# Eric-qi/RDO-PTQ

Measured on AMD Instinct MI355X. Metric: calibration images/sec (Cheng2020 W8A8 task-oriented RDO-PTQ, image-iterations over all units), higher is better.
Workload: dtype f32

## Files before the change

### rdo-ptq_amd/csrc/conv_wgrad.hip

```cpp
#include <utility>

#include "rdo_common.h"

namespace {

typedef float f32x16 __attribute__((ext_vector_type(16)));
typedef float f32x4 __attribute__((ext_vector_type(4)));

constexpr int PK = 32;

struct WgArgs {
    const float* x;
    const float* dy;
    float* slabs;
    int B, H, W, Cin, Ho, Wo, Cout, KH, KW, stride, pad;
    int M, mchunk, nsplit;
    int tiles_co, tiles_ci;
    int square_input;
};

template <int TCO, int TCI, bool VEC>
__global__ __launch_bounds__(256) void conv_wgrad_kernel(WgArgs a) {
    constexpr int WCO = TCO / 2, WCI = TCI / 2;
    constexpr int TM = WCO / 32, TN = WCI / 32;
    constexpr int YQ = TCO / 32, XQ = TCI / 32;
// ... 192 lines not shown
}

int rdo_launch_wgrad_x6(const rdo_conv_desc* d, const float* x, const float* dy, float* slabs, int nsplit, int mchunk, hipStream_t s);
bool rdo_linear_wgrad_h2_ok(const rdo_conv_desc* d, const float* x, const float* dy);
int rdo_launch_linear_wgrad_h2(const rdo_conv_desc* d, const float* x, const float* dy, float* slabs, int nsplit, int mchunk, hipStream_t s);
bool rdo_conv_is_thin(const rdo_conv_desc* d, bool forward);
int rdo_launch_thin_wgrad(const rdo_conv_desc* d, const float* x, const float* dy, float* slabs, int nsplit, hipStream_t s);
bool rdo_conv_is_thincout(const rdo_conv_desc* d, bool forward);
int rdo_thincout_patches(const rdo_conv_desc* d);
int rdo_launch_thincout_wgrad(const rdo_conv_desc* d, const float* x, const float* dy, float* slabs, hipStream_t s);

extern "C" int rdo_conv2d_wgrad_uses_bf16x6(const rdo_conv_desc* d) {
    const bool enabled = rdo::tuning(rdo::T_CONV_X6) != 0;
    if (!d || !enabled || g_force_big == 0) return 0;
    const bool fits = (double)d->B * d->H * d->W * d->Cin * 4.0 < 4.0e9 && (double)d->B * d->Ho * d->Wo * d->Cout * 4.0 < 4.0e9;
    return big_tiles(d) && fits && d->Wo % 4 == 0 && d->Wo >= 16 && d->Cin % 4 == 0 && d->Cout % 4 == 0;
}

extern "C" void rdo_debug_force_wgrad_choice(int big, int nsplit) {
    g_force_big = big;
    g_force_ns = nsplit;
}

extern "C" int rdo_conv2d_wgrad_nsplit(const rdo_conv_desc* d) {
    if (!d) return 1;
    if (g_force_big < 0 && rdo_conv_is_thincout(d, false)) return rdo_thincout_patches(d);
    if (g_force_ns >= 1) return g_force_ns;
    const long M = (long)d->B * d->Ho * d->Wo;
    if (rdo_conv_is_thin(d, false)) {
        const long per = d->KH * d->KW * d->Cin > 4 ? 256 : 512;
        const long cap = d->KH * d->KW * d->Cin > 4 ? 256 : 128;
        const long ns = M / per;
        return (int)(ns < 1 ? 1 : (ns > cap ? cap : ns));
    }
    const long target = big_tiles(d) ? 256 : 1024;
    long ns = target / tiles_total(d);
    const long max_by_m = rdo::ceil_div(M, 128);
    if (ns > max_by_m) ns = max_by_m;
    if (ns < 1) ns = 1;
    const long cap = (g_force_big < 0 && one_tile_many_pixels(d)) ? 256 : ((g_force_big != 0 && rdo_linear_wgrad_h2_ok(d, nullptr, nullptr)) ? 128 : 64);
    if (ns > cap) ns = cap;
    return (int)ns;
}

extern "C" int rdo_conv2d_wgrad(const rdo_conv_desc* d, const float* x, const float* dy, float* slabs, int nsplit,
                                void* stream) {
    RDO_REQUIRE(d && x && dy && slabs, "rdo_conv2d_wgrad: null argument");
    RDO_REQUIRE(nsplit >= 1, "rdo_conv2d_wgrad: nsplit < 1");
    RDO_REQUIRE((long)d->B * d->H * d->W * d->Cin < (1L << 31) && (long)d->B * d->Ho * d->Wo * d->Cout < (1L << 31),
                "rdo_conv2d_wgrad: tensors of 2^31 or more elements are not supported (32-bit staging offsets)");
    WgArgs a;
    a.x = x; a.dy = dy; a.slabs = slabs;
    a.B = d->B; a.H = d->H; a.W = d->W; a.Cin = d->Cin; a.Ho = d->Ho; a.Wo = d->Wo; a.Cout = d->Cout;
    a.KH = d->KH; a.KW = d->KW; a.stride = d->stride; a.pad = d->pad;
    a.M = d->B * d->Ho * d->Wo;
    a.nsplit = nsplit;
    a.mchunk = (int)(rdo::ceil_div(rdo::ceil_div(a.M, nsplit), PK) * PK);
    a.square_input = d->square_input;
    a.tiles_co = a.tiles_ci = 0;
    const bool vec = (d->Cin % 4 == 0) && (d->Cout % 4 == 0) &&
                     ((reinterpret_cast<uintptr_t>(x) | reinterpret_cast<uintptr_t>(dy)) % 16 == 0);
    const bool big = big_tiles(d);
    if (g_force_big < 0 && rdo_conv_is_thincout(d, false) && nsplit == rdo_thincout_patches(d)) {
        const rdo_conv_desc dd = *d;
        return rdo::dispatch([=](hipStream_t s) { return rdo_launch_thincout_wgrad(&dd, x, dy, slabs, s); }, stream, "conv_thincout_wgrad",
// ... 32 lines not shown
```

### rdo-ptq_amd/csrc/conv_wgrad_h2.hip

```cpp
#include <utility>

#include "rdo_common.h"

namespace {

typedef float f32x4acc __attribute__((ext_vector_type(4)));
typedef _Float16 f16x8 __attribute__((ext_vector_type(8)));
typedef short s16x8 __attribute__((ext_vector_type(8)));
typedef short s16x4 __attribute__((ext_vector_type(4)));
constexpr int NP = 2;
typedef unsigned short u16;

__device__ __attribute__((aligned(64))) unsigned g_zero_page_w[16];

constexpr int PK = 32;
constexpr int SUBB = 32 * 128;
constexpr int PLANEB = 3 * SUBB;
constexpr int OPB = NP * PLANEB;
constexpr int STAGEB = 2 * OPB;

struct WgPArgs {
    const u16* xp;
    const u16* yp;
    long xplane, yplane;
    float* slabs;
// ... 409 lines not shown
        Ey = Ex = 0;
    }

    const float fy = lw_pow2(-Ey), fx = lw_pow2(-Ex);
    float* slab = a.slabs + (long)chunk * a.Cout * a.Cin;
#pragma unroll
    for (int j = 0; j < TN; ++j) {
        const int ci = ci0 + wci0 + j * 16 + l16;
        if (ci >= a.Cin) continue;
#pragma unroll
        for (int i = 0; i < TM; ++i)
#pragma unroll
            for (int r = 0; r < 4; ++r) {
                const int co = co0 + wco0 + i * 16 + 4 * lc + r;
                if (co < a.Cout) slab[(long)co * a.Cin + ci] = (acc[i][j][r] * fy) * fx;
            }
    }
}

constexpr int XROWS = 40;
constexpr int XPLANEB = XROWS * 128;
constexpr int STAGE3B = OPB + NP * XPLANEB;

template <int SUB, int RING3, int LSLOT, int PF = 0>
__global__ __launch_bounds__(512, 2) void conv_wgrad_h2r_kernel(WgPArgs a) {
    constexpr int T = 192;
    constexpr int TM = 3, TN = 6;
    constexpr int SLOTB = SUB * STAGE3B;

    extern __shared__ __attribute__((aligned(16))) char smem[];

    const int tid = threadIdx.x, lane = tid & 63, wave = __builtin_amdgcn_readfirstlane(tid >> 6);
    const int l16 = lane & 15, lc = lane >> 4;
    const int wco0 = (wave >> 1) * 48;

    const int nwg = gridDim.x * gridDim.y;
    const int lin = blockIdx.x + gridDim.x * blockIdx.y;
    const int xq = nwg >> 3, xr = nwg & 7, xcd = lin & 7;
    const int lid = (xcd < xr ? xcd * (xq + 1) : xr * (xq + 1) + (xcd - xr) * xq) + (lin >> 3);
    const int chunk = lid / gridDim.y;
    int t = lid - chunk * gridDim.y;
    const int cib = t % a.tiles_ci; t /= a.tiles_ci;
    const int tco = t % a.tiles_co; t /= a.tiles_co;
    const int kh = __builtin_amdgcn_readfirstlane(t);
    const int co0 = tco * T, ci0 = cib * 64;

    const int segs_row = a.Wo / PK;
    const int segs_total = a.B * a.Ho * segs_row;
    const int spc = (segs_total + a.nsplit - 1) / a.nsplit;
    const int sbeg = chunk * spc;
    const int send = min(segs_total, sbeg + spc);
    const int nsegs = send > sbeg ? send - sbeg : 0;
    const int nsteps = (nsegs + SUB - 1) / SUB;

    const int prow8 = (lane >> 1) & 7, dsl = lane >> 4, dhalf = lane & 1;
    constexpr int XP = NP * 5;
    constexpr unsigned OOB = 0xFFFFFFFFu;
    constexpr int RSRC3 = 0x00020000;
    typedef __attribute__((address_space(3))) void lds_void;
    const unsigned ybytes = (unsigned)(a.yplane * 2), xbytes = (unsigned)(a.xplane * 2);
    __amdgpu_buffer_rsrc_t ry[3], rx[2];
    unsigned yvoff[3], xvoff[2];
    int ydst[3], xdst[2];
#pragma unroll
    for (int j = 0; j < 3; ++j) {
        const int k = wave + 8 * j;
        const int plane = k / 12, sub = (k % 12) >> 2, rg = k & 3;
        const int row = 8 * rg + prow8;
        const int ch = co0 + 64 * sub + 16 * dsl + 8 * dhalf;
        ry[j] = __builtin_amdgcn_make_buffer_rsrc((void*)(a.yp + plane * a.yplane), 0, ybytes, RSRC3);
        yvoff[j] = ch < a.Cout ? (unsigned)(((ch >> 4) * a.M + row) * 16 + (ch & 15)) * 2u : OOB;
        ydst[j] = plane * PLANEB + sub * SUBB + rg * 1024;
    }
    int xedge[2];
#pragma unroll
    for (int j = 0; j < 2; ++j) {
        const int k = wave + 8 * j < XP ? wave + 8 * j : wave;
        const int plane = k / 5, rg = k - plane * 5;
        const int row = 8 * rg + prow8;
        const int ch = ci0 + 16 * dsl + 8 * dhalf;
        rx[j] = __builtin_amdgcn_make_buffer_rsrc((void*)(a.xp + plane * a.xplane - 16), 0, xbytes + 32u, RSRC3);
        xvoff[j] = row < PK + 2 ? (unsigned)(((ch >> 4) * a.Min + row) * 16 + (ch & 15)) * 2u : OOB;
        xedge[j] = (row == 0 ? 1 : 0) | (row == PK + 1 ? 2 : 0) | 4;
        xdst[j] = OPB + plane * XPLANEB + rg * 1024;
    }
    int seg = sbeg;
    int cho = (sbeg / segs_row) % a.Ho;
    int cws = sbeg % segs_row;
    unsigned ysoff = (unsigned)sbeg * (PK * 32u);
    unsigned xsoff = (unsigned)(sbeg * PK + (kh - 1) * a.W) * 32u;
    const int row_bad = kh == 0 ? 0 : kh == 2 ? a.Ho - 1 : -1;
    auto dma_seg = [&](char* const dst) {
        const bool live = seg < send;
        const int emask = (cws == 0 ? 1 : 0) | (cws == segs_row - 1 ? 2 : 0) | ((!live || cho == row_bad) ? 4 : 0);
        const unsigned ys = ysoff, xs = xsoff;
        ++seg; ysoff += PK * 32u; xsoff += PK * 32u;
        if (++cws == segs_row) { cws = 0; if (++cho == a.Ho) cho = 0; }
        if (WG_ABL(1)) return;
#pragma unroll
        for (int j = 0; j < 3; ++j)
            __builtin_amdgcn_raw_ptr_buffer_load_lds(ry[j], (lds_void*)(dst + ydst[j]), 16, live ? yvoff[j] : OOB, ys, 0, 0);
#pragma unroll
        for (int j = 0; j < 2; ++j) {
            if (RING3 == 2 && wave + 8 * j >= XP) break;
            __builtin_amdgcn_raw_ptr_buffer_load_lds(rx[j], (lds_void*)(dst + xdst[j]), 16, (xedge[j] & emask) ? OOB : xvoff[j], xs, 0, 0);
        }
    };
    auto dma_stage = [&](int buf) {
#pragma unroll
        for (int u = 0; u < SUB; ++u) dma_seg(smem + buf * SLOTB + u * STAGE3B);
    };

    f32x4acc acc[TM][TN];
#pragma unroll
    for (int i = 0; i < TM; ++i)
#pragma unroll
        for (int j = 0; j < TN; ++j) acc[i][j] = f32x4acc{0.f, 0.f, 0.f, 0.f};

    const int fr = 4 * lc + ((lane >> 2) & 3);
    const int p4 = lane & 3;
    int fa_off[TM], fb_off[TN];
#pragma unroll
    for (int i = 0; i < TM; ++i) {
        const int c = wco0 + 16 * i;
        fa_off[i] = (c >> 6) * SUBB + (fr >> 3) * 1024 + ((c & 63) >> 4) * 256 + (fr & 7) * 32 + p4 * 8;
    }
#pragma unroll
    for (int j = 0; j < TN; ++j) {
        const int jt = 6 * (wave & 1) + j;
        const int row = fr + (jt >> 2);
        fb_off[j] = OPB + (row >> 3) * 1024 + (jt & 3) * 256 + (row & 7) * 32 + p4 * 8;
    }

    constexpr int PA[3] = {1, 0, 0};
    constexpr int PB[3] = {0, 1, 0};

    const bool late = wave >= 4;
    if (nsteps > 0) {
#pragma unroll
        for (int r = 0; r < RING3 - 1; ++r) dma_stage(r);
    }
    if constexpr (PF != 0) {
        static_assert(SUB == 1 && RING3 == 3, "look-ahead variant: one segment per stage, ring of three");
        f16x8 fa[2][NP][TM], fb[2][NP][2];
        auto rd_a = [&](auto pc, const char* st) {
            constexpr int P = decltype(pc)::value;
#pragma unroll
            for (int p = 0; p < NP; ++p)
#pragma unroll
                for (int i = 0; i < TM; ++i) fa[P][p][i] = tr_pair(st + p * PLANEB + fa_off[i]);
        };
        auto rd_b = [&](auto setc, const char* st, int third) {
            constexpr int S = decltype(setc)::value;
#pragma unroll
            for (int p = 0; p < NP; ++p)
#pragma unroll
                for (int j = 0; j < 2; ++j) fb[S][p][j] = tr_pair(st + p * XPLANEB + fb_off[2 * third + j]);
        };
#ifdef RDO_DIAG
        const unsigned long long st_c0 = clock64(), st_r0 = wall_clock64();
#endif
        if (nsteps > 0) {
            asm volatile("s_waitcnt vmcnt(5)" ::: "memory");
            __builtin_amdgcn_s_barrier();
            rd_a(std::integral_constant<int, 0>{}, smem);
            rd_b(std::integral_constant<int, 0>{}, smem, 0);
        }
        auto stage = [&](auto pc, const int s, const int buf) {
            constexpr int P = decltype(pc)::value;
            asm volatile("s_waitcnt vmcnt(0)" ::: "memory");
            __builtin_amdgcn_s_barrier();
            const int nb = buf >= 1 ? buf - 1 : 2;
            const int nx = buf == 2 ? 0 : buf + 1;
            const bool more = s + 2 < nsteps, ahead = s + 1 < nsteps;
            if (more && !late) dma_stage(nb);
            const char* st = smem + buf * SLOTB;
            const char* sn = smem + nx * SLOTB;
            [&]<int... SL>(std::integer_sequence<int, SL...>) {
                (([&] {
                     constexpr int T3 = SL / 3, Q = SL % 3, SET = (T3 + P) & 1;
                     using NS = std::integral_constant<int, SET ^ 1>;
                     if constexpr (Q == 0) {
                         tr_wait();
                         if constexpr (PF == 1) {
                             if constexpr (T3 < 2) rd_b(NS{}, st, T3 + 1);
                             else if (ahead) { rd_a(std::integral_constant<int, P ^ 1>{}, sn); rd_b(NS{}, sn, 0); }
                         }
                     }
                     if constexpr (PF == 1) {
#pragma unroll
                         for (int i = 0; i < TM; ++i)
#pragma unroll
                             for (int j = 0; j < 2; ++j)
                                 acc[i][2 * T3 + j] =
                                     __builtin_amdgcn_mfma_f32_16x16x32_f16(fa[P][PA[Q]][i], fb[SET][PB[Q]][j], acc[i][2 * T3 + j], 0, 0, 0);
                     } else {
                         [&]<int... U>(std::integer_sequence<int, U...>) {
                             (([&] {
                                  constexpr int i = U / 2, j = U % 2, K = Q * 6 + U;
                                  acc[i][2 * T3 + j] =
                                      __builtin_amdgcn_mfma_f32_16x16x32_f16(fa[P][PA[Q]][i], fb[SET][PB[Q]][j], acc[i][2 * T3 + j], 0, 0, 0);
                                  if constexpr (T3 < 2) {
                                      if constexpr (K < 4) fb[SET ^ 1][K / 2][K % 2] = tr_pair(st + (K / 2) * XPLANEB + fb_off[2 * (T3 + 1) + K % 2]);
                                  } else {
                                      if constexpr (K < 6) fa[P ^ 1][K / 3][K % 3] = tr_pair(sn + (K / 3) * PLANEB + fa_off[K % 3]);
                                      else if constexpr (K < 10) fb[SET ^ 1][(K - 6) / 2][(K - 6) % 2] = tr_pair(sn + ((K - 6) / 2) * XPLANEB + fb_off[(K - 6) % 2]);
                                  }
                                  __builtin_amdgcn_sched_barrier(0);
                              }()),
                              ...);
                         }
                         (std::make_integer_sequence<int, 6>{});
                     }
                     __builtin_amdgcn_sched_barrier(0);
                     if constexpr (SL == LSLOT) {
                         if (more && late) dma_stage(nb);
                     }
                     __builtin_amdgcn_sched_barrier(0);
                 }()),
                 ...);
            }
            (std::make_integer_sequence<int, 9>{});
        };
        int buf = 0;
        for (int s = 0; s < nsteps; s += 2) {
            stage(std::integral_constant<int, 0>{}, s, buf);
            buf = buf == 2 ? 0 : buf + 1;
            if (s + 1 < nsteps) {
                stage(std::integral_constant<int, 1>{}, s + 1, buf);
                buf = buf == 2 ? 0 : buf + 1;
            }
        }
        tr_wait();
#ifdef RDO_DIAG
        if (tid == 0 && lin < 256) {
// ... 93 lines not shown
            }
            (std::make_integer_sequence<int, 9>{});
#ifdef RDO_DIAG
            if (phase_on) ph[4] += clock64() - tb;
#endif
        }
        buf = buf + 1 == RING3 ? 0 : buf + 1;
    }
#ifdef RDO_DIAG
    if (tid == 0 && lin < 256) {
        g_wg_stamps[lin * 4 + 0] = clock64() - st_c0; g_wg_stamps[lin * 4 + 1] = wall_clock64() - st_r0;
        g_wg_stamps[lin * 4 + 2] = (unsigned long long)(nsteps * SUB); g_wg_stamps[lin * 4 + 3] = 0;
    }
    if (phase_on && lane == 0 && lin < 256)
        for (int k = 0; k < 6; ++k) g_wg_phase[(lin * 8 + wave) * 8 + k] = ph[k];
#endif
    }
    asm volatile("s_waitcnt vmcnt(0)" ::: "memory");

    const long wsize = (long)a.Cout * 9 * a.Cin;
    float* slab = a.slabs + (long)chunk * wsize;
#pragma unroll
    for (int j = 0; j < TN; ++j) {
        const int jt = 6 * (wave & 1) + j;
        const int tap = kh * 3 + (jt >> 2);
        const int ci = ci0 + (jt & 3) * 16 + l16;
#pragma unroll
        for (int i = 0; i < TM; ++i)
#pragma unroll
            for (int r = 0; r < 4; ++r) {
                const int co = co0 + wco0 + i * 16 + 4 * lc + r;
                if (co < a.Cout) slab[((long)co * 9 + tap) * a.Cin + ci] = acc[i][j][r] * a.inv_scale;
            }
    }
}

}

extern "C" int rdo_conv2d_wgrad_uses_bf16x6(const rdo_conv_desc* d);
extern "C" int rdo_conv2d_wgrad_nsplit(const rdo_conv_desc* d);

extern "C" int rdo_conv2d_wgrad_h2_supported(const rdo_conv_desc* d) {
    if (!d || d->square_input || d->Cin % 16 != 0 || d->Cout % 16 != 0) return 0;
    if ((double)d->B * d->H * d->W * d->Cin >= 2147483648.0 - 64.0 || (double)d->B * d->Ho * d->Wo * d->Cout >= 2147483648.0 - 64.0) return 0;
    return rdo_conv2d_wgrad_uses_bf16x6(d);
}

// ... 16 lines not shown
    a.B = d->B; a.H = d->H; a.W = d->W; a.Cin = d->Cin; a.Ho = d->Ho; a.Wo = d->Wo; a.Cout = d->Cout;
    a.KH = d->KH; a.KW = d->KW; a.stride = d->stride; a.pad = d->pad;
    a.M = d->B * d->Ho * d->Wo;
    a.Min = d->B * d->H * d->W;
    a.xplane = (long)a.Min * a.Cin;
    a.yplane = (long)a.M * a.Cout;
    a.nsplit = nsplit;
    RDO_REQUIRE(x_scale > 0.f && dy_scale > 0.f, "rdo_conv2d_wgrad_h2: scales must be positive powers of two");
    a.inv_scale = 1.f / (x_scale * dy_scale);
#ifdef RDO_DIAG
    a.ablate = rdo::tuning(rdo::T_X6P_ABLATE);
#endif
    long mchunk = rdo::ceil_div(rdo::ceil_div((long)a.M, nsplit), 32) * 32;
    a.mchunk = (int)mchunk;
    RDO_REQUIRE((long)nsplit * mchunk >= a.M, "rdo_conv2d_wgrad_h2: nsplit too small");
    a.tiles_co = (int)rdo::ceil_div(a.Cout, T);
    a.tiles_ci = (int)rdo::ceil_div(a.Cin, T);
    const double flops = 2.0 * a.M * (double)a.Cout * a.Cin * a.KH * a.KW;
    const double bytes = 4.0 * (a.xplane + a.yplane) + 4.0 * nsplit * (double)a.Cout * a.KH * a.KW * a.Cin;
    if (rdo_conv2d_wgrad_h2_supported(d) && rdo::tuning(rdo::T_WGRAD_P3_ROW) && a.KH == 3 && a.KW == 3 && a.stride == 1 && a.pad == 1 && a.Wo % 32 == 0 && a.Cin % 64 == 0 &&
        a.Wo == a.W && a.Ho == a.H && (long)(a.M / 32) >= nsplit) {
        WgPArgs b = a;
        b.tiles_ci = a.Cin / 64;
        const int variant = rdo::tuning(rdo::T_WGRAD_SUB);
        return rdo::dispatch(
            [b, variant](hipStream_t s) {
                auto go = [&](auto subc, auto ringc, auto slotc, auto pfc) -> int {
                    constexpr int SUB = decltype(subc)::value, RING = decltype(ringc)::value, LS = decltype(slotc)::value, PF = decltype(pfc)::value;
                    constexpr size_t lds = (size_t)RING * SUB * STAGE3B;
                    static_assert(lds <= 160 * 1024, "row weight-gradient LDS");
                    static rdo::PerDevice attr;
                    if (!attr.done()) {
                        if (hipFuncSetAttribute(reinterpret_cast<const void*>(conv_wgrad_h2r_kernel<SUB, RING, LS, PF>),
                                                hipFuncAttributeMaxDynamicSharedMemorySize, (int)lds) != hipSuccess)
                            return rdo::set_error(RDO_EHIP, "hipFuncSetAttribute(conv_wgrad_h2r) failed");
                        attr.mark();
                    }
                    dim3 grid((unsigned)b.nsplit, (unsigned)(3 * b.tiles_co * b.tiles_ci));
                    hipLaunchKernelGGL((conv_wgrad_h2r_kernel<SUB, RING, LS, PF>), grid, dim3(512), lds, s, b);
                    return rdo::check_launch("conv_wgrad_h2r");
                };
                using rdo_i1 = std::integral_constant<int, 1>; using rdo_i2 = std::integral_constant<int, 2>; using rdo_i3 = std::integral_constant<int, 3>;
                using rdo_i5 [[maybe_unused]] = std::integral_constant<int, 5>; using rdo_i8 = std::integral_constant<int, 8>;
                using rdo_i0 = std::integral_constant<int, 0>;
                switch (variant) {
                    case 2: return go(rdo_i2{}, rdo_i2{}, rdo_i2{}, rdo_i0{});
                    case 3: return go(rdo_i1{}, rdo_i3{}, rdo_i8{}, rdo_i0{});
                    case 9: return go(rdo_i1{}, rdo_i3{}, rdo_i2{}, rdo_i1{});
                    case 13: return go(rdo_i1{}, rdo_i3{}, rdo_i2{}, rdo_i2{});
#ifdef RDO_DIAG
                    case 4: return go(rdo_i1{}, rdo_i3{}, rdo_i5{}, rdo_i0{});
                    case 5: return go(rdo_i1{}, rdo_i2{}, rdo_i5{}, rdo_i0{});
                    case 6: return go(rdo_i1{}, rdo_i2{}, rdo_i8{}, rdo_i0{});
                    case 7: return go(rdo_i1{}, rdo_i2{}, rdo_i0{}, rdo_i0{});
                    case 8: return go(rdo_i1{}, rdo_i3{}, rdo_i5{}, rdo_i1{});
                    case 10: return go(rdo_i1{}, rdo_i3{}, rdo_i8{}, rdo_i1{});
                    case 11: return go(rdo_i1{}, rdo_i3{}, rdo_i0{}, rdo_i1{});
                    case 12: return go(rdo_i1{}, rdo_i3{}, rdo_i3{}, rdo_i1{});
                    case 14: return go(rdo_i1{}, rdo_i3{}, rdo_i5{}, rdo_i2{});
                    case 15: return go(rdo_i1{}, rdo_i3{}, rdo_i0{}, rdo_i2{});
#endif
                    default: return go(rdo_i1{}, rdo_i2{}, rdo_i2{}, rdo_i0{});
                }
            },
            stream, "conv_wgrad_h2_rows", flops, bytes);
    }
    return rdo::dispatch(
        [a](hipStream_t s) {
            constexpr size_t lds = (size_t)2 * STAGEB;
            static rdo::PerDevice attr;
            if (!attr.done()) {
                if (hipFuncSetAttribute(reinterpret_cast<const void*>(conv_wgrad_h2_kernel), hipFuncAttributeMaxDynamicSharedMemorySize,
                                        (int)lds) != hipSuccess)
                    return rdo::set_error(RDO_EHIP, "hipFuncSetAttribute(conv_wgrad_h2) failed");
                attr.mark();
            }
            dim3 grid((unsigned)a.nsplit, (unsigned)(a.KH * a.KW * a.tiles_co * a.tiles_ci));
            hipLaunchKernelGGL(conv_wgrad_h2_kernel, grid, dim3(512), lds, s, a);
            return rdo::check_launch("conv_wgrad_h2");
        },
        stream, "conv_wgrad_h2_192x192", flops, bytes);
}

static long lw_min_tokens() {
    static const long v = [] { const char* e = getenv("RDO_LIN_WGRAD_H2_MIN"); return e ? atol(e) : 4096L; }();
// ... 43 lines not shown
```

### rdo-ptq_amd/csrc/rdo_common.h

```cpp
#pragma once
#include <hip/hip_runtime.h>

#include <atomic>
#include <cstdarg>
#include <cstdint>
#include <cstdio>
#include <functional>
#include <string>
#include <vector>

#include "../../include/rdo_ptq_hip.h"

namespace rdo {

struct Op {
    std::function<int(hipStream_t)> fn;
    const char* tag;
    double flops;
    double bytes;
};

struct Recorder {
    bool active = false;
    std::vector<Op>* sink = nullptr;
// ... 15 lines not shown
    hipError_t e = hipGetLastError();
    if (e != hipSuccess) return set_error(RDO_EHIP, "%s: %s", what, hipGetErrorString(e));
    return RDO_OK;
}

#define RDO_REQUIRE(cond, ...)                                  \
    do {                                                        \
        if (!(cond)) return rdo::set_error(RDO_EINVAL, __VA_ARGS__); \
    } while (0)

constexpr int kWave = 64;

struct PerDevice {
    std::atomic<uint64_t> bits{0};
    static uint64_t bit() {
        int d = 0;
        (void)hipGetDevice(&d);
        return 1ull << (d & 63);
    }
    bool done() const { return (bits.load(std::memory_order_acquire) & bit()) != 0; }
    void mark() { bits.fetch_or(bit(), std::memory_order_release); }
};

enum Tune { T_WGRAD_X6_W8 = 0, T_CONV_X6, T_FWD_X6_VER, T_XCD, T_X6P_ABLATE, T_GRAPH_UNROLL, T_TAIL_GRID, T_X6P_HALO, T_WGRAD_P3_ROW, T_THIN_MFMA, T_H2_STAGGER, T_ADA_W1_MIN, T_H2_K32, T_WGRAD_SUB, T_H2_N48, T_COUNT };
int tuning(Tune t);

__host__ __device__ inline long frag_index(long e, int Cout, int KH, int KW, int Cin) {
    if (Cin % 16 != 0) return e;
    long t = e / Cin;
    const int ci = (int)(e - t * Cin);
    const int kw = (int)(t % KW);
    t /= KW;
    const int kh = (int)(t % KH);
    const long co = t / KH;
    return (((((long)(ci >> 4) * KH + kh) * KW + kw) * Cout + co) << 4) + (ci & 15);
}
__host__ __device__ inline int group_row(int r, int rows) { return (r & 3) * (rows >> 2) + (r >> 2); }
__host__ __device__ inline long group_row_elem(long e, int rows, long inner) {
    const long r = e / inner;
    return (long)group_row((int)r, rows) * inner + (e - r * inner);
}
inline int64_t ceil_div(int64_t a, int64_t b) { return (a + b - 1) / b; }

constexpr int kGridCap = 2048;
inline unsigned grid_for(long n, int per_thread = 1) {
    const long g = ceil_div(n, 256L * per_thread);
    return (unsigned)(g < 1 ? 1 : (g > kGridCap ? kGridCap : g));
// ... 69 lines not shown
```

### rdo-ptq_amd/csrc/runtime.hip

```cpp
#include "rdo_common.h"

#include <atomic>
#include <cstdlib>
#include <cstring>
#include <mutex>

namespace rdo {

static thread_local std::string g_err;
static thread_local Recorder g_rec;

Recorder& recorder() { return g_rec; }

int set_error(int code, const char* fmt, ...) {
    char buf[512];
    va_list ap;
    va_start(ap, fmt);
    vsnprintf(buf, sizeof buf, fmt, ap);
    va_end(ap);
    g_err = buf;
    return code;
}

namespace {
struct TuneDef { const char* key; const char* env; int dflt; };
constexpr TuneDef kTune[T_COUNT] = {{"wgrad_x6_w8", "RDO_WGX6_W8", 1}, {"conv_x6", "RDO_CONV_X6", 1},
                                    {"fwd_x6_ver", "RDO_X6_VER", 6}, {"xcd", "RDO_XCD", 1},
                                    {"x6p_ablate", "RDO_X6P_ABLATE", 0}, {"graph_unroll", "RDO_GRAPH_UNROLL", 8},
                                    {"tail_grid", "RDO_TAIL_GRID", 1024}, {"x6p_halo", "RDO_X6P_HALO", 1},
                                    {"wgrad_p3_row", "RDO_WGRAD_P3_ROW", 1}, {"thin_mfma", "RDO_THIN_MFMA", 1},
                                    {"h2_stagger", "RDO_H2_STAGGER", 1}, {"ada_w1_min", "RDO_ADA_W1_MIN", 128},
                                    {"h2_k32", "RDO_H2_K32", 3}, {"wgrad_sub", "RDO_WGRAD_SUB", 13}, {"h2_n48", "RDO_H2_N48", 1}};
std::atomic<int> g_tune[T_COUNT];
std::once_flag g_tune_once;
void tune_init() {
    std::call_once(g_tune_once, [] {
        for (int i = 0; i < T_COUNT; ++i) {
            const char* e = getenv(kTune[i].env);
            int v = e ? atoi(e) : kTune[i].dflt;
#ifndef RDO_DIAG
            if (i == T_X6P_ABLATE || (i == T_FWD_X6_VER && v < 5) || (i == T_WGRAD_X6_W8 && v == 0)) v = kTune[i].dflt;
#endif
            g_tune[i].store(v);
        }
    });
}
int tune_index(const char* key) {
    if (!key) return -1;
    for (int i = 0; i < T_COUNT; ++i)
        if (!strcmp(key, kTune[i].key)) return i;
    return -1;
}
}

int tuning(Tune t) {
// ... 291 lines not shown
```

### rdo-ptq_amd/hipops/_lib.py

```python
import ctypes as C
import os

_HERE = os.path.dirname(os.path.abspath(__file__))
LIB_PATH = os.path.join(os.path.dirname(_HERE), "lib", "librdoptq_hip.so")

EPI_NONE, EPI_LRELU, EPI_LRELU_BWD, EPI_GDN, EPI_IGDN, EPI_RELU, EPI_RELU_BWD, EPI_GELU, EPI_GELU_BWD = range(9)
LOG_SLOTS = 32


class ConvDesc(C.Structure):
    _fields_ = [(n, C.c_int32) for n in ("B", "H", "W", "Cin", "Ho", "Wo", "Cout", "KH", "KW", "stride", "pad", "epilogue",
                                         "square_input", "add_residual")]


class AdaDesc(C.Structure):
    _fields_ = [("numel", C.c_int64), ("rows", C.c_int32), ("n_levels", C.c_int32), ("reparam", C.c_int32),
                ("reparam_bound", C.c_float), ("reparam_pedestal", C.c_float), ("KH", C.c_int32), ("KW", C.c_int32),
                ("Cin", C.c_int32)]


class AdaStepItem(C.Structure):
    _fields_ = [("d", AdaDesc), ("w", C.c_void_p), ("delta", C.c_void_p), ("zp", C.c_void_p), ("slabs", C.c_void_p),
                ("nsplit", C.c_int32), ("alpha", C.c_void_p), ("adam_m", C.c_void_p), ("adam_v", C.c_void_p), ("wq", C.c_void_p),
                ("wd", C.c_void_p), ("wq_planes", C.c_void_p), ("wd_planes", C.c_void_p), ("dalpha", C.c_void_p),
# ... 173 lines not shown
    "rdo_uaq_width_scan": (C.c_int, [P, C.c_int32, C.c_int64, C.POINTER(C.c_int32), C.c_int32, P, P, P, P, P, P, P, P]),
    "rdo_uaq_width_scan_workspace": (C.c_int64, [C.c_int32, C.c_int64, C.c_int32]),
}
EXPORTS_BITS = tuple(_SIGS_BITS)
WIDTH_SCAN_MAX_K = 8
WIDTH_SCAN_MIN_BITS, WIDTH_SCAN_MAX_BITS = 2, 16
WIDTH_SCAN_LDS_ROW, WIDTH_SCAN_CHUNK = 8192, 4096
_SIGS_PACK = {
    "rdo_weight_pack": (C.c_int, [P, P, P, P, C.c_int32, C.c_int64, C.c_int32, P, P]),
    "rdo_weight_unpack": (C.c_int, [P, P, P, C.c_int32, C.c_int64, C.c_int32, P, P, P]),
    "rdo_pack_row_words": (C.c_int64, [C.c_int64, C.c_int32]),
}
EXPORTS_PACK = tuple(_SIGS_PACK)
PACK_MIN_BITS, PACK_MAX_BITS = 2, 16

_SIGS_ACTBITS = {
    "rdo_actquant_width_scan": (C.c_int, [P, C.c_int64, C.c_int32, P, C.POINTER(C.c_int32), C.c_int32, P, P, P, P]),
    "rdo_actquant_width_scan_workspace": (C.c_int64, [C.c_int32, C.c_int32]),
}
EXPORTS_ACTBITS = tuple(_SIGS_ACTBITS)
ACT_WIDTH_SCAN_MAX_K = 8
ACT_WIDTH_SCAN_MIN_BITS, ACT_WIDTH_SCAN_MAX_BITS = 2, 16

_lib = None


def lib():
    global _lib
    if _lib is None:
        if not os.path.exists(LIB_PATH):
            raise RuntimeError(f"{LIB_PATH} not found: build it with `python __graft_entry__.py` or "
                               f"`make -C rdo-ptq_amd/csrc` (no CPU fallback exists)")
        import torch
        h = C.CDLL(LIB_PATH)
        for name, (res, args) in (list(_SIGS.items()) + list(_SIGS_GDN.items()) + list(_SIGS_BIAS.items()) + list(_SIGS_BITS.items())
                                  + list(_SIGS_PACK.items()) + list(_SIGS_SUBPEL.items()) + list(_SIGS_ACTBITS.items())):
            fn = getattr(h, name)
            fn.restype, fn.argtypes = res, args
        _lib = h
    return _lib


def check(rc, what=""):
    if rc != 0:
        raise RuntimeError(f"librdoptq_hip {what} failed ({rc}): {lib().rdo_last_error().decode()}")
```

### rdo-ptq_amd/hipops/ops.py

```python
import ctypes as C
import math
import threading

import torch

from . import _args as A
from . import _lib as L


class H2:
    __slots__ = ("t", "scale", "flag")

    def __init__(self, t, scale, flag=None):
        self.t, self.scale = t, float(scale)
        self.flag = flag
        m, e = math.frexp(self.scale)
        if not (self.scale > 0 and m == 0.5):
            raise ValueError(f"H2 scale must be a positive power of two, got {scale}")

    @property
    def device(self):
        return self.t.device


# ... 1517 lines not shown
            "rdo_pixel_shuffle_h2")


def pixel_unshuffle2(x, out=None, out_planes=None):
    B, Hr, Wr, Cc = x.shape
    if out is None and out_planes is None:
        out = torch.empty((B, Hr // 2, Wr // 2, 4 * Cc), device=x.device, dtype=torch.float32)
    _bind_out(out_planes)
    L.check(L.lib().rdo_pixel_unshuffle2(_ptr(x), B, Hr // 2, Wr // 2, Cc, _ptr(out), _ptr(out_planes), _oscale(out_planes), _stream()),
            "rdo_pixel_unshuffle2")
    return out


def wgrad_h2_supported(x_shape, w_shape, stride, pad):
    d = conv_desc(x_shape, w_shape, stride, pad)
    return bool(L.lib().rdo_conv2d_wgrad_h2_supported(C.byref(d)))


def wgrad_h2_layer_supported(x_shape, w_shape, stride, pad):
    d = conv_desc(x_shape, w_shape, stride, pad)
    return bool(L.lib().rdo_conv2d_wgrad_h2_layer_supported(C.byref(d)))


def conv2d_wgrad_h2(xp, x_shape, dyp, w_shape, stride=1, pad=0, slabs=None):
    d = conv_desc(x_shape, w_shape, stride, pad)
    ns = int(L.lib().rdo_conv2d_wgrad_nsplit(C.byref(d))) if slabs is None else slabs.shape[0]
    if slabs is None:
        slabs = torch.empty((ns,) + tuple(w_shape), device=xp.device, dtype=torch.float32)
    L.check(L.lib().rdo_conv2d_wgrad_h2(C.byref(d), _ptr(xp), xp.scale, _ptr(dyp), dyp.scale, _ptr(slabs), ns, _stream()), "rdo_conv2d_wgrad_h2")
    return slabs
```

Before: 21860.

## Add narrow 96-channel output tile variant for row weight-gradient kernel

Adds a TCO=96 template variant of the fp16 row-based 3x3 weight-gradient kernel, where four waves share a 48-column output strip instead of two. A heuristic picks the narrow tile when the 192-wide tiling leaves too few workgroups or too little work per split. The split count is recomputed from the narrower tile count so the grid grows. The aim is better CU occupancy on small or low-Cout layers, at the cost of more x-operand re-loading per output channel and more partial slabs to reduce.

```diff
diff --git a/include/rdo_ptq_wgrad.h b/include/rdo_ptq_wgrad.h
--- /dev/null
+++ b/include/rdo_ptq_wgrad.h
@@ -0,0 +1,15 @@
+#ifndef RDO_PTQ_WGRAD_H
+#define RDO_PTQ_WGRAD_H
+
+#include "rdo_ptq_hip.h"
+
+#ifdef __cplusplus
+extern "C" {
+#endif
+
+int rdo_conv2d_wgrad_h2_tco(const rdo_conv_desc* d);
+
+#ifdef __cplusplus
+}
+#endif
+#endif
diff --git a/rdo-ptq_amd/csrc/conv_wgrad.hip b/rdo-ptq_amd/csrc/conv_wgrad.hip
--- a/rdo-ptq_amd/csrc/conv_wgrad.hip
+++ b/rdo-ptq_amd/csrc/conv_wgrad.hip
@@ -1,6 +1,7 @@
 #include <utility>
 
 #include "rdo_common.h"
+#include "../../include/rdo_ptq_wgrad.h"
 
 namespace {
 
@@ -239,6 +240,34 @@
     g_force_ns = nsplit;
 }
 
+
+static long splits_for_tiles(const rdo_conv_desc* d, long tiles) {
+    const long M = (long)d->B * d->Ho * d->Wo;
+    const long target = big_tiles(d) ? 256 : 1024;
+    long ns = target / tiles;
+    const long max_by_m = rdo::ceil_div(M, 128);
+    if (ns > max_by_m) ns = max_by_m;
+    if (ns < 1) ns = 1;
+    const long cap = (g_force_big < 0 && one_tile_many_pixels(d)) ? 256 : ((g_force_big != 0 && rdo_linear_wgrad_h2_ok(d, nullptr, nullptr)) ? 128 : 64);
+    return ns > cap ? cap : ns;
+}
+
+extern "C" int rdo_conv2d_wgrad_h2_tco(const rdo_conv_desc* d) {
+    const int mode = rdo::tuning(rdo::T_WGRAD_NARROW);
+    if (!d || mode == 0 || g_force_ns >= 1) return 192;
+    const bool rows = d->KH == 3 && d->KW == 3 && d->stride == 1 && d->pad == 1 && d->Wo % 32 == 0 && d->Cin % 64 == 0 && d->Wo == d->W &&
+                      d->Ho == d->H && rdo_conv2d_wgrad_h2_supported(d);
+    if (!rows) return 192;
+    if (mode == 96) return 96;
+    const long segs = (long)d->B * d->Ho * d->Wo / 32;
+    const long ns192 = splits_for_tiles(d, tiles_total(d));
+    if (rdo::ceil_div(segs, ns192) >= 64) return 192;
+    const long tiles96 = 3 * rdo::ceil_div(d->Cout, 96) * (d->Cin / 64);
+    const long ns96 = splits_for_tiles(d, tiles96);
+    if (rdo::ceil_div(segs, ns96) >= 8 && tiles96 * ns96 >= 224) return 96;
+    return 192;
+}
+
 extern "C" int rdo_conv2d_wgrad_nsplit(const rdo_conv_desc* d) {
     if (!d) return 1;
     if (g_force_big < 0 && rdo_conv_is_thincout(d, false)) return rdo_thincout_patches(d);
@@ -250,14 +279,9 @@
         const long ns = M / per;
         return (int)(ns < 1 ? 1 : (ns > cap ? cap : ns));
     }
-    const long target = big_tiles(d) ? 256 : 1024;
-    long ns = target / tiles_total(d);
-    const long max_by_m = rdo::ceil_div(M, 128);
-    if (ns > max_by_m) ns = max_by_m;
-    if (ns < 1) ns = 1;
-    const long cap = (g_force_big < 0 && one_tile_many_pixels(d)) ? 256 : ((g_force_big != 0 && rdo_linear_wgrad_h2_ok(d, nullptr, nullptr)) ? 128 : 64);
-    if (ns > cap) ns = cap;
-    return (int)ns;
+    const int tco = rdo_conv2d_wgrad_h2_tco(d);
+    const long tiles = tco != 192 ? 3 * rdo::ceil_div(d->Cout, tco) * (d->Cin / 64) : (long)tiles_total(d);
+    return (int)splits_for_tiles(d, tiles);
 }
 
 extern "C" int rdo_conv2d_wgrad(const rdo_conv_desc* d, const float* x, const float* dy, float* slabs, int nsplit,
diff --git a/rdo-ptq_amd/csrc/conv_wgrad_h2.hip b/rdo-ptq_amd/csrc/conv_wgrad_h2.hip
--- a/rdo-ptq_amd/csrc/conv_wgrad_h2.hip
+++ b/rdo-ptq_amd/csrc/conv_wgrad_h2.hip
@@ -1,6 +1,7 @@
 #include <utility>
 
 #include "rdo_common.h"
+#include "../../include/rdo_ptq_wgrad.h"
 
 namespace {
 
@@ -456,17 +457,24 @@
 constexpr int XPLANEB = XROWS * 128;
 constexpr int STAGE3B = OPB + NP * XPLANEB;
 
-template <int SUB, int RING3, int LSLOT, int PF = 0>
+template <int SUB, int RING3, int LSLOT, int PF = 0, int TCO = 192>
 __global__ __launch_bounds__(512, 2) void conv_wgrad_h2r_kernel(WgPArgs a) {
-    constexpr int T = 192;
-    constexpr int TM = 3, TN = 6;
-    constexpr int SLOTB = SUB * STAGE3B;
+    static_assert(TCO == 192 || (TCO == 96 && PF == 2), "narrow tiles: the shipped look-ahead stage shape only");
+    constexpr int T = TCO;
+    constexpr int CLOG = TCO == 192 ? 1 : 2;
+    constexpr int TM = 3, TN = 12 >> CLOG;
+    constexpr int CPT = TN / 3;
+    constexpr int YSUBS = (TCO + 63) / 64;
+    constexpr int YPLANEB = YSUBS * SUBB, YOPB = NP * YPLANEB;
+    constexpr int STG = YOPB + NP * XPLANEB;
+    constexpr int YPW = NP * YSUBS * 4 / 8;
+    constexpr int SLOTB = SUB * STG;
 
     extern __shared__ __attribute__((aligned(16))) char smem[];
 
     const int tid = threadIdx.x, lane = tid & 63, wave = __builtin_amdgcn_readfirstlane(tid >> 6);
     const int l16 = lane & 15, lc = lane >> 4;
-    const int wco0 = (wave >> 1) * 48;
+    const int wco0 = (wave >> CLOG) * 48, colg = wave & ((1 << CLOG) - 1);
 
     const int nwg = gridDim.x * gridDim.y;
     const int lin = blockIdx.x + gridDim.x * blockIdx.y;
@@ -497,14 +505,16 @@
     unsigned yvoff[3], xvoff[2];
     int ydst[3], xdst[2];
 #pragma unroll
-    for (int j = 0; j < 3; ++j) {
+    for (int j = 0; j < YPW; ++j) {
         const int k = wave + 8 * j;
-        const int plane = k / 12, sub = (k % 12) >> 2, rg = k & 3;
+        const int plane = k / (4 * YSUBS), sub = (k % (4 * YSUBS)) >> 2, rg = k & 3;
         const int row = 8 * rg + prow8;
         const int ch = co0 + 64 * sub + 16 * dsl + 8 * dhalf;
+        bool chok = ch < a.Cout;
+        if constexpr (TCO % 64 != 0) chok = chok && 64 * sub + 16 * dsl < TCO;
         ry[j] = __builtin_amdgcn_make_buffer_rsrc((void*)(a.yp + plane * a.yplane), 0, ybytes, RSRC3);
-        yvoff[j] = ch < a.Cout ? (unsigned)(((ch >> 4) * a.M + row) * 16 + (ch & 15)) * 2u : OOB;
-        ydst[j] = plane * PLANEB + sub * SUBB + rg * 1024;
+        yvoff[j] = chok ? (unsigned)(((ch >> 4) * a.M + row) * 16 + (ch & 15)) * 2u : OOB;
+        ydst[j] = plane * YPLANEB + sub * SUBB + rg * 1024;
     }
     int xedge[2];
 #pragma unroll
@@ -516,7 +526,7 @@
         rx[j] = __builtin_amdgcn_make_buffer_rsrc((void*)(a.xp + plane * a.xplane - 16), 0, xbytes + 32u, RSRC3);
         xvoff[j] = row < PK + 2 ? (unsigned)(((ch >> 4) * a.Min + row) * 16 + (ch & 15)) * 2u : OOB;
         xedge[j] = (row == 0 ? 1 : 0) | (row == PK + 1 ? 2 : 0) | 4;
-        xdst[j] = OPB + plane * XPLANEB + rg * 1024;
+        xdst[j] = YOPB + plane * XPLANEB + rg * 1024;
     }
     int seg = sbeg;
     int cho = (sbeg / segs_row) % a.Ho;
@@ -532,7 +542,7 @@
         if (++cws == segs_row) { cws = 0; if (++cho == a.Ho) cho = 0; }
         if (WG_ABL(1)) return;
 #pragma unroll
-        for (int j = 0; j < 3; ++j)
+        for (int j = 0; j < YPW; ++j)
             __builtin_amdgcn_raw_ptr_buffer_load_lds(ry[j], (lds_void*)(dst + ydst[j]), 16, live ? yvoff[j] : OOB, ys, 0, 0);
 #pragma unroll
         for (int j = 0; j < 2; ++j) {
@@ -542,7 +552,7 @@
     };
     auto dma_stage = [&](int buf) {
 #pragma unroll
-        for (int u = 0; u < SUB; ++u) dma_seg(smem + buf * SLOTB + u * STAGE3B);
+        for (int u = 0; u < SUB; ++u) dma_seg(smem + buf * SLOTB + u * STG);
     };
 
     f32x4acc acc[TM][TN];
@@ -561,9 +571,9 @@
     }
 #pragma unroll
     for (int j = 0; j < TN; ++j) {
-        const int jt = 6 * (wave & 1) + j;
+        const int jt = TN * colg + j;
         const int row = fr + (jt >> 2);
-        fb_off[j] = OPB + (row >> 3) * 1024 + (jt & 3) * 256 + (row & 7) * 32 + p4 * 8;
+        fb_off[j] = YOPB + (row >> 3) * 1024 + (jt & 3) * 256 + (row & 7) * 32 + p4 * 8;
     }
 
     constexpr int PA[3] = {1, 0, 0};
@@ -576,26 +586,26 @@
     }
     if constexpr (PF != 0) {
         static_assert(SUB == 1 && RING3 == 3, "look-ahead variant: one segment per stage, ring of three");
-        f16x8 fa[2][NP][TM], fb[2][NP][2];
+        f16x8 fa[2][NP][TM], fb[2][NP][CPT];
         auto rd_a = [&](auto pc, const char* st) {
             constexpr int P = decltype(pc)::value;
 #pragma unroll
             for (int p = 0; p < NP; ++p)
 #pragma unroll
-                for (int i = 0; i < TM; ++i) fa[P][p][i] = tr_pair(st + p * PLANEB + fa_off[i]);
+                for (int i = 0; i < TM; ++i) fa[P][p][i] = tr_pair(st + p * YPLANEB + fa_off[i]);
         };
         auto rd_b = [&](auto setc, const char* st, int third) {
             constexpr int S = decltype(setc)::value;
 #pragma unroll
             for (int p = 0; p < NP; ++p)
 #pragma unroll
-                for (int j = 0; j < 2; ++j) fb[S][p][j] = tr_pair(st + p * XPLANEB + fb_off[2 * third + j]);
+                for (int j = 0; j < CPT; ++j) fb[S][p][j] = tr_pair(st + p * XPLANEB + fb_off[CPT * third + j]);
         };
 #ifdef RDO_DIAG
         const unsigned long long st_c0 = clock64(), st_r0 = wall_clock64();
 #endif
         if (nsteps > 0) {
-            asm volatile("s_waitcnt vmcnt(5)" ::: "memory");
+            asm volatile("s_waitcnt vmcnt(%0)" ::"n"(YPW + 2) : "memory");
             __builtin_amdgcn_s_barrier();
             rd_a(std::integral_constant<int, 0>{}, smem);
             rd_b(std::integral_constant<int, 0>{}, smem, 0);
@@ -625,26 +635,27 @@
 #pragma unroll
                          for (int i = 0; i < TM; ++i)
 #pragma unroll
-                             for (int j = 0; j < 2; ++j)
-                                 acc[i][2 * T3 + j] =
-                                     __builtin_amdgcn_mfma_f32_16x16x32_f16(fa[P][PA[Q]][i], fb[SET][PB[Q]][j], acc[i][2 * T3 + j], 0, 0, 0);
+                             for (int j = 0; j < CPT; ++j)
+                                 acc[i][CPT * T3 + j] =
+                                     __builtin_amdgcn_mfma_f32_16x16x32_f16(fa[P][PA[Q]][i], fb[SET][PB[Q]][j], acc[i][CPT * T3 + j], 0, 0, 0);
                      } else {
+                         constexpr int MPS = TM * CPT, NB = NP * CPT;
                          [&]<int... U>(std::integer_sequence<int, U...>) {
                              (([&] {
-                                  constexpr int i = U / 2, j = U % 2, K = Q * 6 + U;
-                                  acc[i][2 * T3 + j] =
-                                      __builtin_amdgcn_mfma_f32_16x16x32_f16(fa[P][PA[Q]][i], fb[SET][PB[Q]][j], acc[i][2 * T3 + j], 0, 0, 0);
+                                  constexpr int i = U / CPT, j = U % CPT, K = Q * MPS + U;
+                                  acc[i][CPT * T3 + j] =
+                                      __builtin_amdgcn_mfma_f32_16x16x32_f16(fa[P][PA[Q]][i], fb[SET][PB[Q]][j], acc[i][CPT * T3 + j], 0, 0, 0);
                                   if constexpr (T3 < 2) {
-                                      if constexpr (K < 4) fb[SET ^ 1][K / 2][K % 2] = tr_pair(st + (K / 2) * XPLANEB + fb_off[2 * (T3 + 1) + K % 2]);
+                                      if constexpr (K < NB) fb[SET ^ 1][K / CPT][K % CPT] = tr_pair(st + (K / CPT) * XPLANEB + fb_off[CPT * (T3 + 1) + K % CPT]);
                                   } else {
-                                      if constexpr (K < 6) fa[P ^ 1][K / 3][K % 3] = tr_pair(sn + (K / 3) * PLANEB + fa_off[K % 3]);
-                                      else if constexpr (K < 10) fb[SET ^ 1][(K - 6) / 2][(K - 6) % 2] = tr_pair(sn + ((K - 6) / 2) * XPLANEB + fb_off[(K - 6) % 2]);
+                                      if constexpr (K < 6) fa[P ^ 1][K / 3][K % 3] = tr_pair(sn + (K / 3) * YPLANEB + fa_off[K % 3]);
+                                      else if constexpr (K < 6 + NB) fb[SET ^ 1][(K - 6) / CPT][(K - 6) % CPT] = tr_pair(sn + ((K - 6) / CPT) * XPLANEB + fb_off[(K - 6) % CPT]);
                                   }
                                   __builtin_amdgcn_sched_barrier(0);
                               }()),
                               ...);
                          }
-                         (std::make_integer_sequence<int, 6>{});
+                         (std::make_integer_sequence<int, MPS>{});
                      }
                      __builtin_amdgcn_sched_barrier(0);
                      if constexpr (SL == LSLOT) {
@@ -784,7 +795,7 @@
     float* slab = a.slabs + (long)chunk * wsize;
 #pragma unroll
     for (int j = 0; j < TN; ++j) {
-        const int jt = 6 * (wave & 1) + j;
+        const int jt = TN * colg + j;
         const int tap = kh * 3 + (jt >> 2);
         const int ci = ci0 + (jt & 3) * 16 + l16;
 #pragma unroll
@@ -847,45 +858,50 @@
         a.Wo == a.W && a.Ho == a.H && (long)(a.M / 32) >= nsplit) {
         WgPArgs b = a;
         b.tiles_ci = a.Cin / 64;
-        const int variant = rdo::tuning(rdo::T_WGRAD_SUB);
+        const int tco = rdo_conv2d_wgrad_h2_tco(d);
+        b.tiles_co = (int)rdo::ceil_div(a.Cout, tco);
+        const int variant = tco == 192 ? rdo::tuning(rdo::T_WGRAD_SUB) : -96;
         return rdo::dispatch(
             [b, variant](hipStream_t s) {
-                auto go = [&](auto subc, auto ringc, auto slotc, auto pfc) -> int {
+                auto go = [&](auto subc, auto ringc, auto slotc, auto pfc, auto tcoc) -> int {
                     constexpr int SUB = decltype(subc)::value, RING = decltype(ringc)::value, LS = decltype(slotc)::value, PF = decltype(pfc)::value;
-                    constexpr size_t lds = (size_t)RING * SUB * STAGE3B;
-                    static_assert(lds <= 160 * 1024, "row weight-gradient LDS");
+                    constexpr int TCO = decltype(tcoc)::value;
+                    constexpr size_t lds = (size_t)RING * SUB * (NP * ((TCO + 63) / 64) * SUBB + NP * XPLANEB);
+                    static_assert(lds <= 160 * 1024 && (TCO != 192 || lds == (size_t)RING * SUB * STAGE3B), "row weight-gradient LDS");
                     static rdo::PerDevice attr;
                     if (!attr.done()) {
-                        if (hipFuncSetAttribute(reinterpret_cast<const void*>(conv_wgrad_h2r_kernel<SUB, RING, LS, PF>),
+                        if (hipFuncSetAttribute(reinterpret_cast<const void*>(conv_wgrad_h2r_kernel<SUB, RING, LS, PF, TCO>),
                                                 hipFuncAttributeMaxDynamicSharedMemorySize, (int)lds) != hipSuccess)
                             return rdo::set_error(RDO_EHIP, "hipFuncSetAttribute(conv_wgrad_h2r) failed");
                         attr.mark();
                     }
                     dim3 grid((unsigned)b.nsplit, (unsigned)(3 * b.tiles_co * b.tiles_ci));
-                    hipLaunchKernelGGL((conv_wgrad_h2r_kernel<SUB, RING, LS, PF>), grid, dim3(512), lds, s, b);
+                    hipLaunchKernelGGL((conv_wgrad_h2r_kernel<SUB, RING, LS, PF, TCO>), grid, dim3(512), lds, s, b);
                     return rdo::check_launch("conv_wgrad_h2r");
                 };
                 using rdo_i1 = std::integral_constant<int, 1>; using rdo_i2 = std::integral_constant<int, 2>; using rdo_i3 = std::integral_constant<int, 3>;
                 using rdo_i5 [[maybe_unused]] = std::integral_constant<int, 5>; using rdo_i8 = std::integral_constant<int, 8>;
                 using rdo_i0 = std::integral_constant<int, 0>;
+                using rdo_i192 = std::integral_constant<int, 192>; using rdo_i96 = std::integral_constant<int, 96>;
                 switch (variant) {
-                    case 2: return go(rdo_i2{}, rdo_i2{}, rdo_i2{}, rdo_i0{});
-                    case 3: return go(rdo_i1{}, rdo_i3{}, rdo_i8{}, rdo_i0{});
-                    case 9: return go(rdo_i1{}, rdo_i3{}, rdo_i2{}, rdo_i1{});
-                    case 13: return go(rdo_i1{}, rdo_i3{}, rdo_i2{}, rdo_i2{});
-#ifdef RDO_DIAG
-                    case 4: return go(rdo_i1{}, rdo_i3{}, rdo_i5{}, rdo_i0{});
-                    case 5: return go(rdo_i1{}, rdo_i2{}, rdo_i5{}, rdo_i0{});
-                    case 6: return go(rdo_i1{}, rdo_i2{}, rdo_i8{}, rdo_i0{});
-                    case 7: return go(rdo_i1{}, rdo_i2{}, rdo_i0{}, rdo_i0{});
-                    case 8: return go(rdo_i1{}, rdo_i3{}, rdo_i5{}, rdo_i1{});
-                    case 10: return go(rdo_i1{}, rdo_i3{}, rdo_i8{}, rdo_i1{});
-                    case 11: return go(rdo_i1{}, rdo_i3{}, rdo_i0{}, rdo_i1{});
-                    case 12: return go(rdo_i1{}, rdo_i3{}, rdo_i3{}, rdo_i1{});
-                    case 14: return go(rdo_i1{}, rdo_i3{}, rdo_i5{}, rdo_i2{});
-                    case 15: return go(rdo_i1{}, rdo_i3{}, rdo_i0{}, rdo_i2{});
-#endif
-                    default: return go(rdo_i1{}, rdo_i2{}, rdo_i2{}, rdo_i0{});
+                    case -96: return go(rdo_i1{}, rdo_i3{}, rdo_i2{}, rdo_i2{}, rdo_i96{});
+                    case 2: return go(rdo_i2{}, rdo_i2{}, rdo_i2{}, rdo_i0{}, rdo_i192{});
+                    case 3: return go(rdo_i1{}, rdo_i3{}, rdo_i8{}, rdo_i0{}, rdo_i192{});
+                    case 9: return go(rdo_i1{}, rdo_i3{}, rdo_i2{}, rdo_i1{}, rdo_i192{});
+                    case 13: return go(rdo_i1{}, rdo_i3{}, rdo_i2{}, rdo_i2{}, rdo_i192{});
+#ifdef RDO_DIAG
+                    case 4: return go(rdo_i1{}, rdo_i3{}, rdo_i5{}, rdo_i0{}, rdo_i192{});
+                    case 5: return go(rdo_i1{}, rdo_i2{}, rdo_i5{}, rdo_i0{}, rdo_i192{});
+                    case 6: return go(rdo_i1{}, rdo_i2{}, rdo_i8{}, rdo_i0{}, rdo_i192{});
+                    case 7: return go(rdo_i1{}, rdo_i2{}, rdo_i0{}, rdo_i0{}, rdo_i192{});
+                    case 8: return go(rdo_i1{}, rdo_i3{}, rdo_i5{}, rdo_i1{}, rdo_i192{});
+                    case 10: return go(rdo_i1{}, rdo_i3{}, rdo_i8{}, rdo_i1{}, rdo_i192{});
+                    case 11: return go(rdo_i1{}, rdo_i3{}, rdo_i0{}, rdo_i1{}, rdo_i192{});
+                    case 12: return go(rdo_i1{}, rdo_i3{}, rdo_i3{}, rdo_i1{}, rdo_i192{});
+                    case 14: return go(rdo_i1{}, rdo_i3{}, rdo_i5{}, rdo_i2{}, rdo_i192{});
+                    case 15: return go(rdo_i1{}, rdo_i3{}, rdo_i0{}, rdo_i2{}, rdo_i192{});
+#endif
+                    default: return go(rdo_i1{}, rdo_i2{}, rdo_i2{}, rdo_i0{}, rdo_i192{});
                 }
             },
             stream, "conv_wgrad_h2_rows", flops, bytes);
diff --git a/rdo-ptq_amd/csrc/rdo_common.h b/rdo-ptq_amd/csrc/rdo_common.h
--- a/rdo-ptq_amd/csrc/rdo_common.h
+++ b/rdo-ptq_amd/csrc/rdo_common.h
@@ -61,7 +61,7 @@
     void mark() { bits.fetch_or(bit(), std::memory_order_release); }
 };
 
-enum Tune { T_WGRAD_X6_W8 = 0, T_CONV_X6, T_FWD_X6_VER, T_XCD, T_X6P_ABLATE, T_GRAPH_UNROLL, T_TAIL_GRID, T_X6P_HALO, T_WGRAD_P3_ROW, T_THIN_MFMA, T_H2_STAGGER, T_ADA_W1_MIN, T_H2_K32, T_WGRAD_SUB, T_H2_N48, T_COUNT };
+enum Tune { T_WGRAD_X6_W8 = 0, T_CONV_X6, T_FWD_X6_VER, T_XCD, T_X6P_ABLATE, T_GRAPH_UNROLL, T_TAIL_GRID, T_X6P_HALO, T_WGRAD_P3_ROW, T_THIN_MFMA, T_H2_STAGGER, T_ADA_W1_MIN, T_H2_K32, T_WGRAD_SUB, T_H2_N48, T_WGRAD_NARROW, T_COUNT };
 int tuning(Tune t);
 
 __host__ __device__ inline long frag_index(long e, int Cout, int KH, int KW, int Cin) {
diff --git a/rdo-ptq_amd/csrc/runtime.hip b/rdo-ptq_amd/csrc/runtime.hip
--- a/rdo-ptq_amd/csrc/runtime.hip
+++ b/rdo-ptq_amd/csrc/runtime.hip
@@ -30,7 +30,8 @@
                                     {"tail_grid", "RDO_TAIL_GRID", 1024}, {"x6p_halo", "RDO_X6P_HALO", 1},
                                     {"wgrad_p3_row", "RDO_WGRAD_P3_ROW", 1}, {"thin_mfma", "RDO_THIN_MFMA", 1},
                                     {"h2_stagger", "RDO_H2_STAGGER", 1}, {"ada_w1_min", "RDO_ADA_W1_MIN", 128},
-                                    {"h2_k32", "RDO_H2_K32", 3}, {"wgrad_sub", "RDO_WGRAD_SUB", 13}, {"h2_n48", "RDO_H2_N48", 1}};
+                                    {"h2_k32", "RDO_H2_K32", 3}, {"wgrad_sub", "RDO_WGRAD_SUB", 13}, {"h2_n48", "RDO_H2_N48", 1},
+                                    {"wgrad_narrow", "RDO_WGRAD_NARROW", 1}};
 std::atomic<int> g_tune[T_COUNT];
 std::once_flag g_tune_once;
 void tune_init() {
diff --git a/rdo-ptq_amd/hipops/_lib.py b/rdo-ptq_amd/hipops/_lib.py
--- a/rdo-ptq_amd/hipops/_lib.py
+++ b/rdo-ptq_amd/hipops/_lib.py
@@ -219,6 +219,11 @@
 ACT_WIDTH_SCAN_MAX_K = 8
 ACT_WIDTH_SCAN_MIN_BITS, ACT_WIDTH_SCAN_MAX_BITS = 2, 16
 
+_SIGS_WGRAD = {
+    "rdo_conv2d_wgrad_h2_tco": (C.c_int, [C.POINTER(ConvDesc)]),
+}
+EXPORTS_WGRAD = tuple(_SIGS_WGRAD)
+
 _lib = None
 
 
@@ -231,7 +236,7 @@
         import torch
         h = C.CDLL(LIB_PATH)
         for name, (res, args) in (list(_SIGS.items()) + list(_SIGS_GDN.items()) + list(_SIGS_BIAS.items()) + list(_SIGS_BITS.items())
-                                  + list(_SIGS_PACK.items()) + list(_SIGS_SUBPEL.items()) + list(_SIGS_ACTBITS.items())):
+                                  + list(_SIGS_PACK.items()) + list(_SIGS_SUBPEL.items()) + list(_SIGS_ACTBITS.items()) + list(_SIGS_WGRAD.items())):
             fn = getattr(h, name)
             fn.restype, fn.argtypes = res, args
         _lib = h
diff --git a/rdo-ptq_amd/hipops/ops.py b/rdo-ptq_amd/hipops/ops.py
--- a/rdo-ptq_amd/hipops/ops.py
+++ b/rdo-ptq_amd/hipops/ops.py
@@ -1563,6 +1563,11 @@
     return bool(L.lib().rdo_conv2d_wgrad_h2_layer_supported(C.byref(d)))
 
 
+def wgrad_h2_tco(x_shape, w_shape, stride, pad):
+    d = conv_desc(x_shape, w_shape, stride, pad)
+    return int(L.lib().rdo_conv2d_wgrad_h2_tco(C.byref(d)))
+
+
 def conv2d_wgrad_h2(xp, x_shape, dyp, w_shape, stride=1, pad=0, slabs=None):
     d = conv_desc(x_shape, w_shape, stride, pad)
     ns = int(L.lib().rdo_conv2d_wgrad_nsplit(C.byref(d))) if slabs is None else slabs.shape[0]
```

Result: no change. 22010 (median of 6 runs) (+0.7%).
